# whh1747012859/Enhanced-UNet

Hardware: AMD Instinct MI355X
Metric: training images/sec at 1024×1024 1-ch→2-cls, 1/2/4/8 MI355X; Dice vs CPU ref (higher is better)
Workload: dtype bf16

## Files before the change

### enhanced-unet_amd/csrc/conv3x3.hip

```cpp
#include <algorithm>
#include <type_traits>

#include "common.h"

EUNET_DEBUG_UNIT(conv3x3)

namespace {

constexpr int BN = 64;
constexpr int NTHR = 256;
constexpr int B_UNITS = 4 * BN * 9;
constexpr int B_LDS_BYTES = B_UNITS * 16;

template <typename T> struct KCh { static constexpr int v = 4 * Vec16<T>::N; };

struct FwdArgs {
  const void* x; int N, H, W, xct, xco, cin;
  const float* isc; const float* ish; int iss;
  const void* wp; int cout_pad, nkc;
  const float* bias;
  void* y; int yct, yco, cout;
  float* stats; int tx, ty, ntiles;
  const void* by; int byct, byco;
  const float* bmean; const float* bistd; const float* bsc; const float* bsh;
// ... 610 lines not shown
      }
  #if CONV_STAMP
      st_ep[2 + 2 * pass] = conv_stamp();
  #endif
      if (pass + 1 < NPASS) __syncthreads();
    }
  }
  if (bnb) {
    float bs1[E], bs2[E];
#pragma unroll
    for (int e = 0; e < E; ++e) {
      float v1 = bp1[e >> 1][e & 1], v2 = bp2[e >> 1][e & 1];
      if constexpr (UPX == 8) {
        v1 += __int_as_float(__builtin_amdgcn_mov_dpp(__float_as_int(v1), 0x128, 0xF, 0xF, false));
        v2 += __int_as_float(__builtin_amdgcn_mov_dpp(__float_as_int(v2), 0x128, 0xF, 0xF, false));
      }
      bs1[e] = xor32_sum(xor16_sum(v1));
      bs2[e] = xor32_sum(xor16_sum(v2));
    }
    __syncthreads();
    float* r2 = (float*)smem;
    if (lane < UPX) {
#pragma unroll
      for (int e = 0; e < E; ++e) {
        r2[(wv * UPX + lane) * 2 * E + e] = bs1[e];
        r2[(wv * UPX + lane) * 2 * E + E + e] = bs2[e];
      }
    }
    __syncthreads();
    if (tid < 2 * BN) {
      const int which = tid / BN, cc = tid % BN, u = cc / E, e = cc % E;
      float t = 0.f;
#pragma unroll
      for (int w = 0; w < NW; ++w) t += r2[(w * UPX + u) * 2 * E + which * E + e];
      if (co0 + cc < a.cout) a.bpart[((long long)tile * 2 + which) * a.cout + co0 + cc] = t;
    }
  }
#if CONV_STAMP
  const unsigned long long st_e = conv_stamp();
  if (tid == 0 && blockIdx.x < STAMP_BLOCKS) {
    unsigned long long* o = g_conv_stamps + (size_t)blockIdx.x * STAMP_N;
    o[0] = st_t0;
    o[1] = st_e - st_t0;
    o[2] = st_stage;
    o[3] = st_mfma;
    o[4] = st_e - st_a;
    o[5] = st_ep[0] - st_a;
    o[6] = st_ep[1] - st_ep[0];
    o[7] = st_ep[2] - st_ep[1];
    o[8] = st_ep[3] - st_ep[2];
    o[9] = st_ep[4] - st_ep[3];
    o[10] = st_e - st_ep[4];
  }
#endif
}


template <typename T>
__device__ __forceinline__ void pack_elem(const float* w, int cout, int cin, int flip, T* wp, int cout_p, int cin_p,
                                          long long id) {
  constexpr int E = Vec16<T>::N, KC = KCh<T>::v;
  const int e = (int)(id % E);
  long long r = id / E;
  const int t = (int)(r % 9); r /= 9;
  const int o = (int)(r % cout_p); r /= cout_p;
  const int qq = (int)(r % 4);
  const int kc = (int)(r / 4);
  const int i = kc * KC + qq * E + e;
  float v = 0.f;
  if (!flip) {
    if (o < cout && i < cin) v = w[((long long)o * cin + i) * 9 + t];
  } else {
    if (o < cin && i < cout) v = w[((long long)i * cin + o) * 9 + (8 - t)];
  }
  Elem<T>::st(wp + id, v);
}

template <typename T>
__global__ void pack_kernel(const float* w, int cout, int cin, int flip, T* wp, int cout_p, int cin_p) {
  const long long id = (long long)blockIdx.x * blockDim.x + threadIdx.x;
  if (id < (long long)cin_p * cout_p * 9) pack_elem<T>(w, cout, cin, flip, wp, cout_p, cin_p, id);
}

struct PackBatch {
  eunet_pack_desc d[EUNET_PACK_MAX];
  int cout_p[EUNET_PACK_MAX], cin_p[EUNET_PACK_MAX];
  int bstart[EUNET_PACK_MAX + 1];
  int n;
};
template <typename T>
__global__ __launch_bounds__(256) void pack_many_kernel(PackBatch b) {
  constexpr int E = Vec16<T>::N, KC = KCh<T>::v;
  const int bid = blockIdx.x;
  int k = 0;
  for (int i = 1; i < b.n; ++i) k = bid >= b.bstart[i] ? i : k;
  const eunet_pack_desc& d = b.d[k];
  const int cout_p = b.cout_p[k];
  const long long u = (long long)(bid - b.bstart[k]) * 256 + threadIdx.x;
  if (u >= (long long)b.cin_p[k] * cout_p * 9 / E) return;
  long long r = u;
  const int t = (int)(r % 9); r /= 9;
  const int o = (int)(r % cout_p); r /= cout_p;
  const int qq = (int)(r % 4);
  const int kc = (int)(r / 4);
  const int i0 = kc * KC + qq * E;
  float v[E];
  bool ok[E];
#pragma unroll
  for (int e = 0; e < E; ++e) {
    const int i = i0 + e;
    ok[e] = d.flip ? (o < d.cin && i < d.cout) : (o < d.cout && i < d.cin);
    const long long src = !ok[e] ? 0 : d.flip ? ((long long)i * d.cin + o) * 9 + (8 - t) : ((long long)o * d.cin + i) * 9 + t;
    v[e] = d.w[src];
  }
#pragma unroll
  for (int e = 0; e < E; ++e) asm volatile("" : "+v"(v[e]));
#pragma unroll
  for (int e = 0; e < E; ++e) v[e] = ok[e] ? v[e] : 0.f;
  *(uint4*)((T*)d.wp + u * E) = Vec16<T>::pack(v);
}

struct WgArgs {
  const void* x; int N, H, W, xct, xco, cin;
  const float* isc; const float* ish; int iss;
  const void* dy; int dct, dco, cout;
  float* dw; float* db;
  int tx, ty, ntiles, per_split, nsplit;
};

__device__ __forceinline__ int wd_swz(int p) { return p & 6; }

__device__ __forceinline__ void wg_map(int b, int nsplit, int ncob, int ncib, int& split, int& cob, int& cib) {
  const int total = nsplit * ncob * ncib, full = total & ~7;
  const int L = b < full ? (b & 7) * (full >> 3) + (b >> 3) : b;
  cib = L % ncib;
  const int r = L / ncib;
  cob = r % ncob;
  split = r / ncob;
}

constexpr int KCW = 64;
constexpr int DTH = 8, DTW = 16;
constexpr int DHW = DTW + 2;
constexpr int DHPX = (DTH + 2) * DHW;
constexpr int DPL = 384;
constexpr int DWX = 4 * DPL * 16;
constexpr int DWD = DTH * DTW * 64 * 2;
constexpr int DSTAGE = DWX + DWD;
constexpr int DWX_ITERS = 4 * DPL / NTHR;
constexpr int DWD_ITERS = DTH * DTW * 8 / NTHR;
static_assert(4 * DPL == NTHR * DWX_ITERS && DTH * DTW * 8 == NTHR * DWD_ITERS, "whole wave-instructions");
static_assert(2 * DHPX <= DPL && DPL % 16 == 0, "a pair plane holds the halo, bank-row aligned");
static_assert(2 * DSTAGE <= 80 * 1024, "two stages per block, two blocks per CU");
static_assert(DPL > NTHR, "dma_x: one pair-plane boundary per wave-instruction range at most");

__device__ __forceinline__ void dma16_lds(u32x4 rsrc, uint32_t voff, uint32_t lds) {
  asm volatile("s_mov_b32 m0, %0\n\tbuffer_load_dwordx4 %1, %2, 0 offen lds"
               :: "s"(lds), "v"(voff), "s"(rsrc) : "memory", "m0");
}
__device__ __forceinline__ u32x4 rsrc_of(const void* base, uint32_t bytes) {
  const unsigned long long b = (unsigned long long)base;
  return (u32x4){(uint32_t)__builtin_amdgcn_readfirstlane((int)(uint32_t)b),
                 (uint32_t)__builtin_amdgcn_readfirstlane((int)(uint32_t)(b >> 32)),
                 (uint32_t)__builtin_amdgcn_readfirstlane((int)bytes), 0x00020000u};
}

__global__ __launch_bounds__(NTHR, 2) void conv3x3_wgrad_bf16_kernel(WgArgs a) {
  __shared__ __attribute__((aligned(16))) char wst[2 * DSTAGE];
  const int tid = threadIdx.x, lane = tid & 63, wv = tid >> 6;
  int split, cob, kc;
  wg_map(blockIdx.x, a.nsplit, cdiv(a.cout, 64), cdiv(a.cin, KCW), split, cob, kc);
  const int co0 = cob * 64;
  const int t_begin = split * a.per_split;
  const int t_end = min(a.ntiles, t_begin + a.per_split);
  EUNET_DASSERT(split < a.nsplit && co0 < a.cout && kc * KCW < a.cin && t_begin < a.ntiles);
  const int tpi = a.tx * a.ty;
  const int g = lane >> 4, i16 = lane & 15, q4 = i16 >> 2, p4 = i16 & 3;
  const int pcol = 4 * (g & 1) + q4;
  const int sw16 = (((p4 >> 1) ^ wd_swz(pcol)) * 8 + 4 * (p4 & 1)) * 2;

  f32x4 acc[9][4];
#pragma unroll
  for (int t = 0; t < 9; ++t)
#pragma unroll
    for (int c = 0; c < 4; ++c) acc[t][c] = (f32x4){0.f, 0.f, 0.f, 0.f};
  f32x2 dbv[4];
#pragma unroll
  for (int e = 0; e < 4; ++e) dbv[e] = (f32x2){0.f, 0.f};
  if (blockIdx.x & 1) __builtin_amdgcn_s_sleep(40);

  const uint32_t lds0 = (uint32_t)(size_t)(__attribute__((address_space(3))) char*)wst;
  const uint32_t wlds = lds0 + (uint32_t)__builtin_amdgcn_readfirstlane(wv) * 1024u;
  const int dp = tid >> 3, dcol = dp & (DTW - 1), drow = dp >> 4, du = (tid & 7) ^ wd_swz(dp);
  const bool dch_ok = co0 + du * 8 < a.cout;
  const uint32_t rstep = (uint32_t)(a.W * a.dct) * 2u;
  const uint32_t dlane = (uint32_t)((dcol * a.dct + a.dco + co0 + du * 8) * 2) + (uint32_t)drow * rstep;
  const uint32_t dslice = (uint32_t)(a.H * a.W * a.dct) * 2u, xslice = (uint32_t)(a.H * a.W * a.xct) * 2u;
  auto dma_d = [&](int st, int n, int y0, int x0) {
    const u32x4 dr = rsrc_of((const bf16_t*)a.dy + (long long)n * a.H * a.W * a.dct, dslice);
    const bool xok = dch_ok & (dcol < a.W - x0);
    const uint32_t rb = (uint32_t)((y0 * a.W + x0) * a.dct) * 2u;
    const uint32_t l = wlds + (uint32_t)(st * DSTAGE + DWX);
#pragma unroll
    for (int i = 0; i < DWD_ITERS; ++i) {
      const bool ok = xok & (y0 + 2 * i + drow < a.H);
      const uint32_t off = dlane + rb + 2u * i * rstep;
      EUNET_DASSERT(!ok || off + 16u <= dslice);
      dma16_lds(dr, ok ? off : FWD_OOB, l + 4096u * i);
    }
  };
  auto dma_x = [&](int st, int n, int y0, int x0) {
    const u32x4 xr = rsrc_of((const bf16_t*)a.x + (long long)n * a.H * a.W * a.xct, xslice);
    const int tb = ((y0 - 1) * a.W + (x0 - 1)) * a.xct + a.xco + kc * KCW;
    const uint32_t l = wlds + (uint32_t)(st * DSTAGE);
    int t = tid;
    asm volatile("" : "+v"(t));
#pragma unroll
    for (int i = 0; i < DWX_ITERS; ++i) {
      const int k = NTHR * i / DPL, tk = DPL * (k + 1) - NTHR * i;
      const bool bump = tk < NTHR && t >= tk;
      const int pr = k + bump, r = t + NTHR * i - DPL * pr;
      const int oc = 2 * pr + (r & 1), hp = r >> 1;
      const int hy = (int)((uint32_t)hp / DHW), hx = hp - hy * DHW;
      const bool ok = ((uint32_t)hp < (uint32_t)DHPX) & ((uint32_t)(y0 - 1 + hy) < (uint32_t)a.H) &
                      ((uint32_t)(x0 - 1 + hx) < (uint32_t)a.W) & (kc * KCW + oc * 8 < a.cin);
      const uint32_t off = (uint32_t)(tb + (hy * a.W + hx) * a.xct + oc * 8) * 2u;
      EUNET_DASSERT(!ok || off + 16u <= xslice);
      dma16_lds(xr, ok ? off : FWD_OOB, l + 4096u * i);
    }
  };
  const int xo = 2 * wv + (lane & 1);
  const bool xo_ok = kc * KCW + xo * 8 < a.cin;
  auto load_aff = [&](int n, f32x4* sc) {
    const float* ps = a.isc + (long long)n * a.iss + kc * KCW + xo * 8;
    const float* ph = a.ish + (long long)n * a.iss + kc * KCW + xo * 8;
    const f32x4 z = {0.f, 0.f, 0.f, 0.f};
    sc[0] = xo_ok ? *(const f32x4*)ps : z;
    sc[1] = xo_ok ? *(const f32x4*)(ps + 4) : z;
    sc[2] = xo_ok ? *(const f32x4*)ph : z;
    sc[3] = xo_ok ? *(const f32x4*)(ph + 4) : z;
  };
  auto bnrelu_x = [&](char* S, int y0, int x0, const f32x4* sc) {
    if (!xo_ok) return;
    const float scv[8] = {sc[0][0], sc[0][1], sc[0][2], sc[0][3], sc[1][0], sc[1][1], sc[1][2], sc[1][3]};
    const float shv[8] = {sc[2][0], sc[2][1], sc[2][2], sc[2][3], sc[3][0], sc[3][1], sc[3][2], sc[3][3]};
    char* const plane = S + (wv * DPL + lane) * 16;
    constexpr int G = 3, NI = (2 * DHPX + 63) / 64;
    static_assert(NI % G == 0, "bnrelu_x groups");
    static_assert((3 * DPL + 63 + 64 * (NI - 1) + 1) * 16 <= DSTAGE, "bnrelu_x: group reads stay inside the stage");
#pragma unroll 1
    for (int i0 = 0; i0 < NI; i0 += G) {
      u32x4 w[G];
      bool ok[G];
#pragma unroll
      for (int j = 0; j < G; ++j) {
        const int hp = (lane >> 1) + 32 * (i0 + j), hy = hp / DHW, hx = hp - hy * DHW;
        const int yy = y0 + hy - 1, xx = x0 + hx - 1;
        ok[j] = (hp < DHPX) & ((uint32_t)yy < (uint32_t)a.H) & ((uint32_t)xx < (uint32_t)a.W);
        w[j] = *(const u32x4*)(plane + 64 * (i0 + j) * 16);
      }
#pragma unroll
      for (int j = 0; j < G; ++j) {
        u32x4 o;
#pragma unroll
        for (int d = 0; d < 4; ++d) {
          const f32x2 x = {__uint_as_float(w[j][d] << 16), __uint_as_float(w[j][d] & 0xFFFF0000u)};
          const f32x2 r = __builtin_elementwise_fma(x, (f32x2){scv[2 * d], scv[2 * d + 1]}, (f32x2){shv[2 * d], shv[2 * d + 1]});
          const s16x2 b = __builtin_bit_cast(s16x2, pk_bf16(r[0], r[1]));
          o[d] = __builtin_bit_cast(uint32_t, __builtin_elementwise_max(b, (s16x2){0, 0}));
        }
        if (ok[j]) *(u32x4*)(plane + 64 * (i0 + j) * 16) = o;
      }
    }
  };
  int tn = t_begin / tpi, tyi = (t_begin - tn * tpi) / a.tx, txi = t_begin - tn * tpi - tyi * a.tx;
  const bool tf = a.isc != nullptr;
  {
    const int n = __builtin_amdgcn_readfirstlane(tn);
    dma_x(0, n, __builtin_amdgcn_readfirstlane(tyi) * DTH, __builtin_amdgcn_readfirstlane(txi) * DTW);
    dma_d(0, n, __builtin_amdgcn_readfirstlane(tyi) * DTH, __builtin_amdgcn_readfirstlane(txi) * DTW);
  }
  for (int tile = t_begin; tile < t_end; ++tile) {
    const int st = (tile - t_begin) & 1;
    char* const S = wst + st * DSTAGE;
    const int n = __builtin_amdgcn_readfirstlane(tn);
    const int y0 = __builtin_amdgcn_readfirstlane(tyi) * DTH, x0 = __builtin_amdgcn_readfirstlane(txi) * DTW;
    if (++txi == a.tx) {
      txi = 0;
      if (++tyi == a.ty) { tyi = 0; ++tn; }
    }
    f32x4 sc[4];
    if (tf) load_aff(n, sc);
    __builtin_amdgcn_s_waitcnt(0x0F70);
    __syncthreads();
    if (tile + 1 < t_end) {
      const int n1 = __builtin_amdgcn_readfirstlane(tn);
      const int y1 = __builtin_amdgcn_readfirstlane(tyi) * DTH, x1 = __builtin_amdgcn_readfirstlane(txi) * DTW;
      dma_x(st ^ 1, n1, y1, x1);
      dma_d(st ^ 1, n1, y1, x1);
    }
    if (tf) {
      bnrelu_x(S, y0, x0, sc);
      asm volatile("s_waitcnt lgkmcnt(0)" ::: "memory");
    }
    const char* const Xs = S;
    const char* const Ds = S + DWX;
    if (a.db != nullptr && kc == 0) {
      const bf16_t* d = (const bf16_t*)Ds;
#pragma unroll
      for (int i = 0; i < DTH * DTW / 32; ++i) {
        const int px = (tid >> 3) + 32 * i;
        const u32x4 w = *(const u32x4*)(d + px * 64 + ((tid & 7) ^ wd_swz(px)) * 8);
#pragma unroll
        for (int e = 0; e < 4; ++e) dbv[e] += (f32x2){__uint_as_float(w[e] << 16), __uint_as_float(w[e] & 0xFFFF0000u)};
      }
    }
    __builtin_amdgcn_s_setprio(1);
#pragma unroll 1
    for (int ks = 0; ks < DTH * DTW / 32; ++ks) {
      bf16x8 af[4];
      const int pxa = ks * 32 + 16 * (g >> 1) + pcol;
#pragma unroll
      for (int ct = 0; ct < 4; ++ct) {
        const int uo = (32 * ct) ^ sw16;
        const s16x4 lo = __builtin_amdgcn_ds_read_tr16_b64_v4i16(LDS_PTR(s16x4, Ds + pxa * 128 + uo));
        const s16x4 hi = __builtin_amdgcn_ds_read_tr16_b64_v4i16(LDS_PTR(s16x4, Ds + (pxa + 8) * 128 + uo));
        af[ct] = cat_bf16x4(lo, hi);
      }
      const int hrow = 2 * ks + (g >> 1);
#pragma unroll
      for (int t = 0; t < 9; ++t) {
        const int ky = t / 3, kx = t - ky * 3;
        const int hp = (hrow + ky) * DHW + pcol + kx;
        const char* base = Xs + (wv * DPL + 2 * hp + (p4 >> 1)) * 16 + (p4 & 1) * 8;
        const s16x4 lo = __builtin_amdgcn_ds_read_tr16_b64_v4i16(LDS_PTR(s16x4, base));
        const s16x4 hi = __builtin_amdgcn_ds_read_tr16_b64_v4i16(LDS_PTR(s16x4, base + 16 * 16));
        const bf16x8 bfr = cat_bf16x4(lo, hi);
#pragma unroll
        for (int ct = 0; ct < 4; ++ct)
          acc[t][ct] = __builtin_amdgcn_mfma_f32_16x16x32_bf16(af[ct], bfr, acc[t][ct], 0, 0, 0);
      }
    }
    __builtin_amdgcn_s_setprio(0);
  }
  float* out = a.dw + (long long)split * a.cout * 9 * a.cin;
  const int ci = kc * KCW + wv * 16 + i16;
#pragma unroll
  for (int t = 0; t < 9; ++t)
#pragma unroll
    for (int ct = 0; ct < 4; ++ct)
#pragma unroll
      for (int e = 0; e < 4; ++e) {
        const int co = co0 + ct * 16 + g * 4 + e;
        if (co < a.cout && ci < a.cin) {
          EUNET_DASSERT(split < a.nsplit);
          out[((long long)co * 9 + t) * a.cin + ci] = acc[t][ct][e];
        }
      }
  if (a.db != nullptr && kc == 0) {
    float* dbred = (float*)wst;
    __syncthreads();
#pragma unroll
    for (int e = 0; e < 8; ++e) dbred[(tid >> 3) * 64 + (tid & 7) * 8 + e] = dbv[e >> 1][e & 1];
    __syncthreads();
    if (tid < 64 && co0 + tid < a.cout) {
      float t = 0.f;
      for (int r = 0; r < 32; ++r) t += dbred[r * 64 + tid];
      a.db[(long long)split * a.cout + co0 + tid] = t;
    }
  }
}

constexpr int WF_TH = 4, WF_TW = 32;
constexpr int WF_HW = WF_TW + 2;
constexpr int WF_HP = (WF_TH + 2) * WF_HW;
constexpr int WF_CI = 32, WF_CO = 64;
constexpr int WF_XU = WF_HP * WF_CI / 4;
constexpr int WF_DU = WF_TH * WF_TW * WF_CO / 4;
constexpr int WF_XI = (WF_XU + NTHR - 1) / NTHR;
constexpr int WF_DI = WF_DU / NTHR;
constexpr int WF_XS = (WF_CI / 16) * WF_HP * 16;
constexpr int WF_LDS = (WF_XS + (WF_CO / 16) * WF_TH * WF_TW * 16 + 4 * 64) * 4;
static_assert(2 * WF_LDS <= 160 * 1024, "fp32 wgrad: two blocks per CU");

__global__ __launch_bounds__(NTHR, 2) void conv3x3_wgrad_f32_kernel(WgArgs a) {
  extern __shared__ __attribute__((aligned(16))) char smem[];
  float* Xs = (float*)smem;
  float* Ds = Xs + WF_XS;
  float* dbs = Ds + (WF_CO / 16) * WF_TH * WF_TW * 16;
  const int tid = threadIdx.x, lane = tid & 63, wv = tid >> 6;
  int split, cob, cib;
  wg_map(blockIdx.x, a.nsplit, cdiv(a.cout, WF_CO), cdiv(a.cin, WF_CI), split, cob, cib);
  const int co0 = cob * WF_CO, ci0 = cib * WF_CI;
  const int t_begin = split * a.per_split;
  const int t_end = min(a.ntiles, t_begin + a.per_split);
  const int tpi = a.tx * a.ty;
  const int kq = lane >> 4, li = lane & 15;
  const int ct0 = 2 * (wv >> 1), cit = wv & 1;
  const bool do_db = a.db != nullptr && cib == 0;

  f32x4 acc[2][9];
#pragma unroll
  for (int j = 0; j < 2; ++j)
#pragma unroll
    for (int t = 0; t < 9; ++t) acc[j][t] = (f32x4){0.f, 0.f, 0.f, 0.f};
  float dbacc = 0.f;

  uint4 rx[WF_XI], rd[WF_DI];
  unsigned rok = 0;
  auto gload = [&](int tile) {
    const int n = tile / tpi, trem = tile - n * tpi;
    const int y0 = (trem / a.tx) * WF_TH, x0 = (trem % a.tx) * WF_TW;
    rok = 0;
#pragma unroll
    for (int i = 0; i < WF_XI; ++i) {
      const int u = tid + i * NTHR;
      const int m = u & 3, hp = (u >> 2) % WF_HP, tl = (u >> 2) / WF_HP;
      const int hy = hp / WF_HW, hx = hp - hy * WF_HW;
      const int yy = y0 + hy - 1, xx = x0 + hx - 1, c = ci0 + tl * 16 + 4 * m;
      rx[i] = make_uint4(0, 0, 0, 0);
      if (u < WF_XU && yy >= 0 && yy < a.H && xx >= 0 && xx < a.W && c < a.cin) {
        rx[i] = *(const uint4*)((const float*)a.x + ((long long)(n * a.H + yy) * a.W + xx) * a.xct + a.xco + c);
        rok |= 1u << i;
      }
    }
#pragma unroll
    for (int i = 0; i < WF_DI; ++i) {
      const int u = tid + i * NTHR;
      const int m = u & 3, px = (u >> 2) % (WF_TH * WF_TW), tl = (u >> 2) / (WF_TH * WF_TW);
      const int yy = y0 + px / WF_TW, xx = x0 + px % WF_TW, co = co0 + tl * 16 + 4 * m;
      rd[i] = make_uint4(0, 0, 0, 0);
      if (yy < a.H && xx < a.W && co < a.cout)
        rd[i] = *(const uint4*)((const float*)a.dy + ((long long)(n * a.H + yy) * a.W + xx) * a.dct + a.dco + co);
    }
  };
  auto lwrite = [&](int tile) {
    const int n = tile / tpi;
#pragma unroll
    for (int i = 0; i < WF_XI; ++i) {
      const int u = tid + i * NTHR;
      if (u >= WF_XU) continue;
      uint4 v = rx[i];
      if (a.isc != nullptr && ((rok >> i) & 1u)) {
        const int m = u & 3, tl = (u >> 2) / WF_HP, c = ci0 + tl * 16 + 4 * m + n * a.iss;
        float f[4];
        Vec16<float>::unpack(v, f);
#pragma unroll
        for (int e = 0; e < 4; ++e) f[e] = fmaxf(fmaf(f[e], a.isc[c + e], a.ish[c + e]), 0.f);
        v = Vec16<float>::pack(f);
      }
      *(uint4*)(Xs + 4 * u) = v;
    }
#pragma unroll
    for (int i = 0; i < WF_DI; ++i) *(uint4*)(Ds + 4 * (tid + i * NTHR)) = rd[i];
  };

  if (t_begin < t_end) gload(t_begin);
  for (int tile = t_begin; tile < t_end; ++tile) {
    __syncthreads();
    lwrite(tile);
    __syncthreads();
    if (tile + 1 < t_end) gload(tile + 1);
    if (do_db) {
#pragma unroll 4
      for (int i = 0; i < WF_TH * WF_TW / 4; ++i) {
        const int px = (tid >> 6) + 4 * i, co = tid & 63;
        dbacc += Ds[((co >> 4) * WF_TH * WF_TW + px) * 16 + (co & 15)];
      }
    }
    const float* xb = Xs + cit * WF_HP * 16 + li;
    const float* d0 = Ds + (ct0 * WF_TH * WF_TW) * 16 + li;
    const float* d1 = d0 + WF_TH * WF_TW * 16;
#pragma unroll 2
    for (int ks = 0; ks < WF_TH * WF_TW / 4; ++ks) {
      const int px = 4 * ks + kq, r = px / WF_TW, c = px - r * WF_TW;
      const float a0 = d0[px * 16], a1 = d1[px * 16];
#pragma unroll
      for (int t = 0; t < 9; ++t) {
        const int ky = t / 3, kx = t - 3 * ky;
        const float bv = xb[((r + ky) * WF_HW + c + kx) * 16];
        acc[0][t] = __builtin_amdgcn_mfma_f32_16x16x4f32(a0, bv, acc[0][t], 0, 0, 0);
        acc[1][t] = __builtin_amdgcn_mfma_f32_16x16x4f32(a1, bv, acc[1][t], 0, 0, 0);
      }
    }
  }
  float* out = a.dw + (long long)split * a.cout * 9 * a.cin;
  const int ci = ci0 + cit * 16 + li;
#pragma unroll
  for (int j = 0; j < 2; ++j)
#pragma unroll
    for (int t = 0; t < 9; ++t)
#pragma unroll
      for (int i = 0; i < 4; ++i) {
        const int co = co0 + (ct0 + j) * 16 + 4 * kq + i;
        if (co < a.cout && ci < a.cin) out[((long long)co * 9 + t) * a.cin + ci] = acc[j][t][i];
// ... 291 lines not shown
```

### enhanced-unet_amd/eunet/engine.py

```python
from __future__ import annotations

from typing import Dict, Optional

import torch

from . import kprof, ops
from ._lib import EunetError

ENCODER_SCOPE = "conv3x3.encoder_train"

BLOCKS = ("enc1", "enc2", "enc3", "enc4", "dec4", "dec3", "dec2")
UPCONVS = ("up4", "up3", "up2")
BN_EPS = 1e-5
BN_MOMENTUM = 0.1
class Grad1x1:

    def __init__(self, w, k, gz):
        self.w, self.k, self.gz = w, k, gz


class GradPool:

    def __init__(self, gpool, gskip):
        self.gpool, self.gskip = gpool, gskip
# ... 127 lines not shown
        S = self.forward_trunk(x, training)
        P, B = self._P(), self._B()
        N, H, W, K, dev = S["N"], S["H"], S["W"], self.K, x.device
        z = S["z"]
        hws = _e(ops.head_workspace_bytes(N, H, W, K, self.dtype), torch.uint8, dev)
        hmean = _e(64, torch.float32, dev) if training else None
        hinv = _e(64, torch.float32, dev) if training else None
        out2h = _e((N, K, 2 * H, 2 * W), torch.float32, dev) if want == "out2h" else None
        logits = _e((N, K, H, W), torch.float32, dev) if want == "logits" else None
        ops.head_fwd(z, N, H, W, K, P["enhance.0.weight"], P["enhance.0.bias"], P["enhance.1.weight"],
                     P["enhance.1.bias"], P["enhance.3.weight"].reshape(K, 64).contiguous(), P["enhance.3.bias"],
                     training, BN_EPS, BN_MOMENTUM, B["enhance.1.running_mean"], B["enhance.1.running_var"],
                     hmean, hinv, out2h, logits, hws, dtype=self.dtype)
        if training:
            guard = ops.update_guard(dev)
            if guard is None:
                B["enhance.1.num_batches_tracked"].add_(1)
            else:
                B["enhance.1.num_batches_tracked"].add_(guard.eq(0).long().reshape(()))
        S.update(hmean=hmean, hinv=hinv, want=want)
        return (logits if want == "logits" else out2h), S

    def forward_trunk(self, x: torch.Tensor, training: bool):
        if not x.is_cuda:
            raise EunetError("EnhancedUNet (eunet) runs on the GPU only; no CPU fallback")
        N, Cin, H, W = x.shape
        if Cin != self.cin:
            raise ValueError(f"expected {self.cin} input channels, got {Cin}")
        if H % 8 or W % 8:
            raise ValueError("H and W must be multiples of 8 (the reference pads to /32)")
        P, B = self._P(), self._B()
        dt, dev, b, K = self.dtype, x.device, self.base, self.K
        ch = [b, 2 * b, 4 * b, 8 * b]
        lv = [(H >> i, W >> i) for i in range(4)]
        S = {}
        wps = self._pack_all(P, training)
        S["wp"] = wps
        if self.transpose:
            S["up"] = {u: ops.upconv2x2_pack(P[f"{self.prefix}{u}.weight"], dt) for u in UPCONVS}
        xin = _e((N, H, W, Cin), dt, dev)
        ops.nchw_to_nhwc(x.contiguous().float(), xin)
        cat4 = _e((N, *lv[2], ch[3] + ch[2]), dt, dev)
        cat3 = _e((N, *lv[1], ch[2] + ch[1]), dt, dev)
        cat2 = _e((N, *lv[0], ch[1] + ch[0]), dt, dev)
        p1 = _e((N, *lv[1], ch[0]), dt, dev)
        p2 = _e((N, *lv[2], ch[1]), dt, dev)
        p3 = _e((N, *lv[3], ch[2]), dt, dev)
        S.update(xin=xin, cat4=cat4, cat3=cat3, cat2=cat2, p1=p1, p2=p2, p3=p3)

        def consume_pool(nm, cat, coff, pooled):
            s = S[nm]
            ops.bnrelu_pool(ops.act(s["yb"]), s["bnb"]["scale"], s["bnb"]["shift"],
                            ops.act(cat, coff, s["yb"].shape[3]), ops.act(pooled))

        def consume_up(nm, cat, up):
            s = S[nm]
            if self.transpose:
                ops.bnrelu_upconv2x2(ops.act(s["yb"]), s["bnb"]["scale"], s["bnb"]["shift"], S["up"][up],
                                     P[f"{self.prefix}{up}.bias"], ops.act(cat, 0, s["yb"].shape[3]))
                return
            ops.bnrelu_upsample(ops.act(s["yb"]), s["bnb"]["scale"], s["bnb"]["shift"],
                                ops.act(cat, 0, s["yb"].shape[3]))

        S["enc1"] = self._block_fwd("enc1", ops.act(xin), training, P, B, small=True, wps=wps)
        consume_pool("enc1", cat2, ch[1], p1)
        S["enc2"] = self._block_fwd("enc2", ops.act(p1), training, P, B, small=False, wps=wps)
        consume_pool("enc2", cat3, ch[2], p2)
        S["enc3"] = self._block_fwd("enc3", ops.act(p2), training, P, B, small=False, wps=wps)
        consume_pool("enc3", cat4, ch[3], p3)
        S["enc4"] = self._block_fwd("enc4", ops.act(p3), training, P, B, small=False, wps=wps)
        consume_up("enc4", cat4, "up4")
        S["dec4"] = self._block_fwd("dec4", ops.act(cat4), training, P, B, small=False, wps=wps)
        consume_up("dec4", cat3, "up3")
        S["dec3"] = self._block_fwd("dec3", ops.act(cat3), training, P, B, small=False, wps=wps)
        consume_up("dec3", cat2, "up2")
        S["dec2"] = self._block_fwd("dec2", ops.act(cat2), training, P, B, small=False, wps=wps)
        s = S["dec2"]
        z = _e((N, H, W, K), torch.float32, dev)
        ops.bnrelu_conv1x1(ops.act(s["yb"]), s["bnb"]["scale"], s["bnb"]["shift"],
                           P[self.prefix + "dec1.weight"].reshape(K, b).contiguous(), P[self.prefix + "dec1.bias"], K, z)
        S.update(z=z, N=N, H=H, W=W)
        return S

    def _block_bwd(self, nm, G, S, P, sink, need_gx: bool, small: bool, gred=(None, 0)):
        with kprof.scope(ENCODER_SCOPE if nm.startswith("enc") else None):
            return self._block_bwd_impl(nm, G, S, P, sink, need_gx, small, gred)

    def _block_bwd_impl(self, nm, G: "torch.Tensor | Grad1x1 | GradPool", S, P, sink: GradSink, need_gx: bool,
                        small: bool, gred=(None, 0)):
        p = f"{self.prefix}{nm}"
        s = S[nm]
        ya, yb, bna, bnb, X = s["ya"], s["yb"], s["bna"], s["bnb"], s["X"]
        N, H, W, C = yb.shape
        dev, dt = yb.device, self.dtype

        def bn_back(prefix, g, y, bn, part=None, tiles=0):
            if isinstance(g, (Grad1x1, GradPool)):
                dbeta, dgamma = sink.slot(prefix + ".bias", (C,)), sink.slot(prefix + ".weight", (C,))
                ops.colsum(part, tiles, 2 * C, dbeta, split=C, out_hi=dgamma)
                gy = torch.empty_like(y)
                if isinstance(g, Grad1x1):
                    ops.bn_bwd_apply_1x1(ops.act(y), g.w, g.k, g.gz, bn["mean"], bn["invstd"], bn["scale"],
                                         bn["shift"], dbeta, dgamma, ops.act(gy))
                else:
                    ops.bn_bwd_apply_pool(g.gpool, g.gskip, ops.act(y), bn["mean"], bn["invstd"], bn["scale"],
                                          bn["shift"], dbeta, dgamma, ops.act(gy))
                return gy
            if part is None:
                tiles = ops.bn_bwd_tiles(ops.act(y))
                part = _e(tiles * 2 * C, torch.float32, dev)
                ops.bn_bwd_reduce(ops.act(g), ops.act(y), bn["mean"], bn["invstd"], bn["scale"],
                                  bn["shift"], part)
            dbeta, dgamma = sink.slot(prefix + ".bias", (C,)), sink.slot(prefix + ".weight", (C,))
            ops.colsum(part, tiles, 2 * C, dbeta, split=C, out_hi=dgamma)
            gy = torch.empty_like(y)
            ops.bn_bwd_apply(ops.act(g), ops.act(y), bn["mean"], bn["invstd"], bn["scale"],
                             bn["shift"], dbeta, dgamma, ops.act(gy))
            return gy

        main = torch.cuda.current_stream(dev)
        side = side_stream(dev) if self.overlap_wgrad else None

        def wgrad(conv, xa: ops.Act, gy, scale=None, shift=None, small_conv=False, on_main=False):
            dw = sink.slot(conv + ".weight", (C, xa.c, 3, 3))
            db = sink.slot(conv + ".bias", (C,))
            if side is None or on_main:
                return wgrad_on_stream(xa, gy, dw, db, scale, shift, small_conv)
            self._wait(side, main)
            with torch.cuda.stream(side):
                wgrad_on_stream(xa, gy, dw, db, scale, shift, small_conv)
            for t in (gy, xa._keep, dw, db):
                t.record_stream(side)

        def wgrad_on_stream(xa: ops.Act, gy, dw, db, scale=None, shift=None, small_conv=False):
            cin = xa.c
            gya = ops.act(gy)
            if small_conv:
                ns = ops.conv_small_wgrad_splits(gya)
            else:
                ns = ops.conv3x3_wgrad_splits(gya, cin, dt)
            dwp = _e(ns * C * 9 * cin, torch.float32, dev)
            dbp = _e(ns * C, torch.float32, dev)
            if small_conv:
                ops.conv_small_wgrad(xa, gya, dwp, dbp, ns)
            else:
                ops.conv3x3_wgrad(xa, gya, dwp, dbp, ns, scale=scale, shift=shift)
            ops.wgrad_reduce(dwp, dbp, ns, C, cin, 9, dw, db)

        def packed(conv):
            wpt = S["wp"].get(conv + ".weight^T") if S.get("wp") else None
            return wpt if wpt is not None else ops.conv3x3_pack(P[conv + ".weight"], dt, flip=True)

        gyb = bn_back(p + ".4", G, yb, bnb, part=gred[0], tiles=gred[1])
        wpt = packed(p + ".3")
        gaa = torch.empty_like(ya)
        ctiles = ops.conv3x3_tiles(ops.act(gaa))
        cpart = _e(ctiles * 2 * C, torch.float32, dev)
        ops.conv3x3_dgrad_bnbwd(ops.act(gyb), wpt, ops.act(gaa), ops.act(ya), bna["mean"], bna["invstd"],
                                bna["scale"], bna["shift"], cpart)
        gya = bn_back(p + ".1", gaa, ya, bna, part=cpart, tiles=ctiles)
        if s.get("za") is not None:
            wgrad(p + ".3", ops.act(s["za"]), gyb)
        else:
            wgrad(p + ".3", ops.act(ya), gyb, bna["scale"], bna["shift"])
        del gyb
        wgrad(p + ".0", X, gya, small_conv=small, on_main=not need_gx)
        del gaa
        names = [f"{p}.{i}.{w}" for i in (0, 1, 3, 4) for w in ("weight", "bias")]
        if side is None:
            sink.ready(names)
        else:
            self._wait(side, main)
            with torch.cuda.stream(side):
                sink.ready(names)
        if not need_gx:
            return None
        wpt = packed(p + ".0")
        gx = _e((N, H, W, X.c), dt, dev)
        ops.conv3x3_dgrad(ops.act(gya), wpt, ops.act(gx))
        return gx

    def backward(self, S, g_out: torch.Tensor, sink: Optional[GradSink] = None):
        P = self._P()
        N, H, W, K, b = S["N"], S["H"], S["W"], self.K, self.base
        dev, dt = g_out.device, self.dtype
        ch = [b, 2 * b, 4 * b, 8 * b]
        sink = sink or GradSink(dev)
        g_out = g_out.contiguous().float()
        gz = _e((N, H, W, K), torch.float32, dev)
        hws = _e(ops.head_workspace_bytes(N, H, W, K, dt), torch.uint8, dev)
        gw1 = sink.slot("enhance.0.weight", (64, K, 3, 3))
        gb1 = sink.slot("enhance.0.bias", (64,))
        gg = sink.slot("enhance.1.weight", (64,))
        gbt = sink.slot("enhance.1.bias", (64,))
        gw2 = sink.slot("enhance.3.weight", (K, 64, 1, 1))
        gb2 = sink.slot("enhance.3.bias", (K,))
        glog = g_out if S["want"] == "logits" else None
        gout2h = g_out if S["want"] == "out2h" else None
        ops.head_bwd(S["z"], N, H, W, K, P["enhance.0.weight"], P["enhance.0.bias"], P["enhance.1.weight"],
                     P["enhance.1.bias"], P["enhance.3.weight"].reshape(K, 64).contiguous(), S["hmean"], S["hinv"],
                     glog, gout2h, gz, gw1, gb1, gg, gbt, gw2, gb2, hws, dtype=dt)
        sink.ready(["enhance.0.weight", "enhance.0.bias", "enhance.1.weight", "enhance.1.bias",
                    "enhance.3.weight", "enhance.3.bias"])
        self.backward_trunk(S, gz, sink)
        return sink.finish()

    def backward_trunk(self, S, gz: torch.Tensor, sink: GradSink):
        P = self._P()
        N, H, W, K, b = S["N"], S["H"], S["W"], self.K, self.base
        dev, dt = gz.device, self.dtype
        ch = [b, 2 * b, 4 * b, 8 * b]
        pre = self.prefix

        def bnr_args(nm):
            s = S[nm]
            return (ops.act(s["yb"]), s["bnb"]["mean"], s["bnb"]["invstd"], s["bnb"]["scale"], s["bnb"]["shift"])

        def upconv_bwd(ghi: ops.Act, glo: torch.Tensor, nm, up):
            s = S[nm]
            C = glo.shape[3]
            ops.upconv2x2_dgrad(ghi, S["up"][up], ops.act(glo))
            names = [f"{pre}{up}.weight", f"{pre}{up}.bias"]
            dw, db = sink.slot(names[0], (C, C, 2, 2)), sink.slot(names[1], (C,))

            def wgrad():
                ya = ops.act(s["yb"])
                ns = ops.upconv2x2_wgrad_splits(ya, dt)
                dwp = _e(ns * 4 * C * C, torch.float32, dev)
                dbp = _e(ns * 4 * C, torch.float32, dev)
                ops.upconv2x2_wgrad(ya, s["bnb"]["scale"], s["bnb"]["shift"], ghi, dwp, dbp, ns)
                ops.wgrad_reduce(dwp, None, ns, C, C, 4, dw, None)
                ops.colsum(dbp, ns * 4, C, db)
                sink.ready(names)

            if not self.overlap_wgrad:
                wgrad()
                return None, 0
            main, side = torch.cuda.current_stream(dev), side_stream(dev)
            self._wait(side, main)
            with torch.cuda.stream(side):
                wgrad()
            for t in (ghi._keep, s["yb"], dw, db):
                t.record_stream(side)
            return None, 0

        def up_bwd(ghi: ops.Act, glo: torch.Tensor, nm, up):
            if self.transpose:
                return upconv_bwd(ghi, glo, nm, up)
            rows = ops.upsample_bwd_bnr_rows(ops.act(glo))
            if not rows:
                ops.upsample_bwd(ghi, ops.act(glo))
                return None, 0
            part = _e(rows * 2 * glo.shape[3], torch.float32, dev)
            ops.upsample_bwd_bnr(ghi, ops.act(glo), *bnr_args(nm), part)
            return part, rows

        def pool_bwd(act_saved: ops.Act, gpool: ops.Act, gskip: ops.Act, shape, nm):
            rows = ops.pool_bwd_add_bnr_rows(act_saved)
            if not rows:
                gout = _e(shape, dt, dev)
                ops.pool_bwd_add(act_saved, gpool, gskip, ops.act(gout))
                return gout, (None, 0)
            part = _e(rows * 2 * shape[3], torch.float32, dev)
            if self.pool_recompute:
                ops.pool_bwd_add_bnr(act_saved, gpool, gskip, None, *bnr_args(nm), part)
                return GradPool(gpool, gskip), (part, rows)
            gout = _e(shape, dt, dev)
            ops.pool_bwd_add_bnr(act_saved, gpool, gskip, ops.act(gout), *bnr_args(nm), part)
            return gout, (part, rows)

        s2 = S["dec2"]
        yb_act = ops.act(s2["yb"])
        tiles = ops.conv1x1_bwd_tiles(yb_act)
        part = _e(tiles * (K * b + K), torch.float32, dev)
        w1 = P[pre + "dec1.weight"].reshape(K, b).contiguous()
        bnb2 = s2["bnb"]
        bpart = _e(tiles * 2 * b, torch.float32, dev)
        if self.dec1_recompute:
            gd2 = Grad1x1(w1, K, gz)
            ops.conv1x1_bwd_bnr(yb_act, bnb2["scale"], bnb2["shift"], w1, K, gz, None, part,
                                bnb2["mean"], bnb2["invstd"], bpart)
        else:
            gd2 = torch.empty_like(s2["yb"])
            ops.conv1x1_bwd_bnr(yb_act, bnb2["scale"], bnb2["shift"], w1, K, gz, ops.act(gd2), part,
                                bnb2["mean"], bnb2["invstd"], bpart)
        red2 = (bpart, tiles)
        ops.colsum(part, tiles, K * b + K, sink.slot(pre + "dec1.weight", (K, b, 1, 1)), split=K * b,
                   out_hi=sink.slot(pre + "dec1.bias", (K,)))
        sink.ready([pre + "dec1.weight", pre + "dec1.bias"])
        g_cat2 = self._block_bwd("dec2", gd2, S, P, sink, need_gx=True, small=False, gred=red2)
        del gd2
        g_d3 = _e((N, H >> 1, W >> 1, ch[1]), dt, dev)
        red = up_bwd(ops.act(g_cat2, 0, ch[1]), g_d3, "dec3", "up2")
        g_cat3 = self._block_bwd("dec3", g_d3, S, P, sink, need_gx=True, small=False, gred=red)
        del g_d3
        g_d4 = _e((N, H >> 2, W >> 2, ch[2]), dt, dev)
        red = up_bwd(ops.act(g_cat3, 0, ch[2]), g_d4, "dec4", "up3")
        g_cat4 = self._block_bwd("dec4", g_d4, S, P, sink, need_gx=True, small=False, gred=red)
        del g_d4
        g_e4 = _e((N, H >> 3, W >> 3, ch[3]), dt, dev)
        red = up_bwd(ops.act(g_cat4, 0, ch[3]), g_e4, "enc4", "up4")
        g_p3 = self._block_bwd("enc4", g_e4, S, P, sink, need_gx=True, small=False, gred=red)
        del g_e4
        g_e3, red = pool_bwd(ops.act(S["cat4"], ch[3], ch[2]), ops.act(g_p3), ops.act(g_cat4, ch[3], ch[2]),
                             (N, H >> 2, W >> 2, ch[2]), "enc3")
        del g_p3, g_cat4
        g_p2 = self._block_bwd("enc3", g_e3, S, P, sink, need_gx=True, small=False, gred=red)
        del g_e3
        g_e2, red = pool_bwd(ops.act(S["cat3"], ch[2], ch[1]), ops.act(g_p2), ops.act(g_cat3, ch[2], ch[1]),
                             (N, H >> 1, W >> 1, ch[1]), "enc2")
        del g_p2, g_cat3
        g_p1 = self._block_bwd("enc2", g_e2, S, P, sink, need_gx=True, small=False, gred=red)
        del g_e2
        g_e1, red = pool_bwd(ops.act(S["cat2"], ch[1], ch[0]), ops.act(g_p1), ops.act(g_cat2, ch[1], ch[0]),
                             (N, H, W, ch[0]), "enc1")
        del g_p1, g_cat2
        self._block_bwd("enc1", g_e1, S, P, sink, need_gx=False, small=True, gred=red)
# ... 24 lines not shown
```

Measured before the change: 192.8.

## Reuse halo rows across vertically consecutive wgrad tiles and reorder tile walk

The conv3x3 wgrad kernel now walks tiles column-major (down y first), so consecutive tiles share two halo rows. Those rows are no longer re-DMA'd or re-normalised, and the top-row input fragments are carried in registers between k-steps and across tiles. Each wave now copies its own pair plane, a separate BN-ReLU path skips bounds checks for interior tiles, and the engine issues one wgrad earlier when no input gradient is needed. The aim is to cut global loads, LDS reads and BN-ReLU work, at the cost of more live registers and more complex correctness conditions.

```diff
diff --git a/enhanced-unet_amd/csrc/conv3x3.hip b/enhanced-unet_amd/csrc/conv3x3.hip
--- a/enhanced-unet_amd/csrc/conv3x3.hip
+++ b/enhanced-unet_amd/csrc/conv3x3.hip
@@ -786,7 +786,8 @@
 static_assert(4 * DPL == NTHR * DWX_ITERS && DTH * DTW * 8 == NTHR * DWD_ITERS, "whole wave-instructions");
 static_assert(2 * DHPX <= DPL && DPL % 16 == 0, "a pair plane holds the halo, bank-row aligned");
 static_assert(2 * DSTAGE <= 80 * 1024, "two stages per block, two blocks per CU");
-static_assert(DPL > NTHR, "dma_x: one pair-plane boundary per wave-instruction range at most");
+static_assert(DPL == 64 * DWX_ITERS, "dma_x: a wave copies its own pair plane in whole wave-instructions");
+static_assert(2 * 2 * DHW >= 64 && 2 * 2 * DHW < 128, "dma_x: halo rows 0, 1 end inside wave-instruction 1");
 
 __device__ __forceinline__ void dma16_lds(u32x4 rsrc, uint32_t voff, uint32_t lds) {
   asm volatile("s_mov_b32 m0, %0\n\tbuffer_load_dwordx4 %1, %2, 0 offen lds"
@@ -843,24 +844,25 @@
       dma16_lds(dr, ok ? off : FWD_OOB, l + 4096u * i);
     }
   };
-  auto dma_x = [&](int st, int n, int y0, int x0) {
+  auto dma_x = [&](int st, int n, int y0, int x0, bool start) {
     const u32x4 xr = rsrc_of((const bf16_t*)a.x + (long long)n * a.H * a.W * a.xct, xslice);
     const int tb = ((y0 - 1) * a.W + (x0 - 1)) * a.xct + a.xco + kc * KCW;
-    const uint32_t l = wlds + (uint32_t)(st * DSTAGE);
-    int t = tid;
+    const uint32_t l = lds0 + (uint32_t)(st * DSTAGE) + (uint32_t)__builtin_amdgcn_readfirstlane(wv) * (DPL * 16u);
+    const int hp_min = start ? 0 : 2 * DHW;
+    int t = lane;
     asm volatile("" : "+v"(t));
+    const int oc = 2 * wv + (t & 1);
 #pragma unroll
     for (int i = 0; i < DWX_ITERS; ++i) {
-      const int k = NTHR * i / DPL, tk = DPL * (k + 1) - NTHR * i;
-      const bool bump = tk < NTHR && t >= tk;
-      const int pr = k + bump, r = t + NTHR * i - DPL * pr;
-      const int oc = 2 * pr + (r & 1), hp = r >> 1;
+      if (i == 0 && !start) continue;
+      const int hp = (t >> 1) + 32 * i;
       const int hy = (int)((uint32_t)hp / DHW), hx = hp - hy * DHW;
-      const bool ok = ((uint32_t)hp < (uint32_t)DHPX) & ((uint32_t)(y0 - 1 + hy) < (uint32_t)a.H) &
+      const bool ok = (hp >= hp_min) & ((uint32_t)hp < (uint32_t)DHPX) & ((uint32_t)(y0 - 1 + hy) < (uint32_t)a.H) &
                       ((uint32_t)(x0 - 1 + hx) < (uint32_t)a.W) & (kc * KCW + oc * 8 < a.cin);
       const uint32_t off = (uint32_t)(tb + (hy * a.W + hx) * a.xct + oc * 8) * 2u;
       EUNET_DASSERT(!ok || off + 16u <= xslice);
-      dma16_lds(xr, ok ? off : FWD_OOB, l + 4096u * i);
+      EUNET_DASSERT(l + 1024u * i + 1024u <= lds0 + (uint32_t)(st * DSTAGE + DWX));
+      dma16_lds(xr, ok ? off : FWD_OOB, l + 1024u * i);
     }
   };
   const int xo = 2 * wv + (lane & 1);
@@ -874,24 +876,29 @@
     sc[2] = xo_ok ? *(const f32x4*)ph : z;
     sc[3] = xo_ok ? *(const f32x4*)(ph + 4) : z;
   };
-  auto bnrelu_x = [&](char* S, int y0, int x0, const f32x4* sc) {
-    if (!xo_ok) return;
+  auto bnrelu_rows = [&](char* S, int y0, int x0, const f32x4* sc, bool start, auto inside) {
     const float scv[8] = {sc[0][0], sc[0][1], sc[0][2], sc[0][3], sc[1][0], sc[1][1], sc[1][2], sc[1][3]};
     const float shv[8] = {sc[2][0], sc[2][1], sc[2][2], sc[2][3], sc[3][0], sc[3][1], sc[3][2], sc[3][3]};
     char* const plane = S + (wv * DPL + lane) * 16;
     constexpr int G = 3, NI = (2 * DHPX + 63) / 64;
     static_assert(NI % G == 0, "bnrelu_x groups");
     static_assert((3 * DPL + 63 + 64 * (NI - 1) + 1) * 16 <= DSTAGE, "bnrelu_x: group reads stay inside the stage");
+    const int hp_min = start ? 0 : 2 * DHW;
 #pragma unroll 1
     for (int i0 = 0; i0 < NI; i0 += G) {
       u32x4 w[G];
       bool ok[G];
 #pragma unroll
       for (int j = 0; j < G; ++j) {
-        const int hp = (lane >> 1) + 32 * (i0 + j), hy = hp / DHW, hx = hp - hy * DHW;
-        const int yy = y0 + hy - 1, xx = x0 + hx - 1;
-        ok[j] = (hp < DHPX) & ((uint32_t)yy < (uint32_t)a.H) & ((uint32_t)xx < (uint32_t)a.W);
-        w[j] = *(const u32x4*)(plane + 64 * (i0 + j) * 16);
+        const int hp = (lane >> 1) + 32 * (i0 + j);
+        ok[j] = (hp >= hp_min) & (hp < DHPX);
+        if (!decltype(inside)::value) {
+          const int hy = hp / DHW, hx = hp - hy * DHW;
+          const int yy = y0 + hy - 1, xx = x0 + hx - 1;
+          ok[j] &= ((uint32_t)yy < (uint32_t)a.H) & ((uint32_t)xx < (uint32_t)a.W);
+        }
+        w[j] = (u32x4){0u, 0u, 0u, 0u};
+        if (start || i0 + j > 0) w[j] = *(const u32x4*)(plane + 64 * (i0 + j) * 16);
       }
 #pragma unroll
       for (int j = 0; j < G; ++j) {
@@ -907,21 +914,28 @@
       }
     }
   };
-  int tn = t_begin / tpi, tyi = (t_begin - tn * tpi) / a.tx, txi = t_begin - tn * tpi - tyi * a.tx;
+  auto bnrelu_x = [&](char* S, int y0, int x0, const f32x4* sc, bool start) {
+    if (!xo_ok) return;
+    if (y0 >= 1 && y0 + DTH < a.H && x0 >= 1 && x0 + DTW < a.W) bnrelu_rows(S, y0, x0, sc, start, std::true_type{});
+    else bnrelu_rows(S, y0, x0, sc, start, std::false_type{});
+  };
+  int tn = t_begin / tpi, txi = (t_begin - tn * tpi) / a.ty, tyi = t_begin - tn * tpi - txi * a.ty;
   const bool tf = a.isc != nullptr;
   {
     const int n = __builtin_amdgcn_readfirstlane(tn);
-    dma_x(0, n, __builtin_amdgcn_readfirstlane(tyi) * DTH, __builtin_amdgcn_readfirstlane(txi) * DTW);
+    dma_x(0, n, __builtin_amdgcn_readfirstlane(tyi) * DTH, __builtin_amdgcn_readfirstlane(txi) * DTW, true);
     dma_d(0, n, __builtin_amdgcn_readfirstlane(tyi) * DTH, __builtin_amdgcn_readfirstlane(txi) * DTW);
   }
+  bf16x8 cf[3], c1[3];
   for (int tile = t_begin; tile < t_end; ++tile) {
     const int st = (tile - t_begin) & 1;
     char* const S = wst + st * DSTAGE;
     const int n = __builtin_amdgcn_readfirstlane(tn);
     const int y0 = __builtin_amdgcn_readfirstlane(tyi) * DTH, x0 = __builtin_amdgcn_readfirstlane(txi) * DTW;
-    if (++txi == a.tx) {
-      txi = 0;
-      if (++tyi == a.ty) { tyi = 0; ++tn; }
+    const bool start = tile == t_begin || y0 == 0;
+    if (++tyi == a.ty) {
+      tyi = 0;
+      if (++txi == a.tx) { txi = 0; ++tn; }
     }
     f32x4 sc[4];
     if (tf) load_aff(n, sc);
@@ -930,15 +944,28 @@
     if (tile + 1 < t_end) {
       const int n1 = __builtin_amdgcn_readfirstlane(tn);
       const int y1 = __builtin_amdgcn_readfirstlane(tyi) * DTH, x1 = __builtin_amdgcn_readfirstlane(txi) * DTW;
-      dma_x(st ^ 1, n1, y1, x1);
+      dma_x(st ^ 1, n1, y1, x1, y1 == 0);
       dma_d(st ^ 1, n1, y1, x1);
     }
     if (tf) {
-      bnrelu_x(S, y0, x0, sc);
+      bnrelu_x(S, y0, x0, sc, start);
       asm volatile("s_waitcnt lgkmcnt(0)" ::: "memory");
     }
     const char* const Xs = S;
     const char* const Ds = S + DWX;
+    const char* const xlane = Xs + (wv * DPL + 2 * pcol + (p4 >> 1)) * 16 + (p4 & 1) * 8;
+    auto xfrag = [&](const char* base) {
+      const s16x4 lo = __builtin_amdgcn_ds_read_tr16_b64_v4i16(LDS_PTR(s16x4, base));
+      const s16x4 hi = __builtin_amdgcn_ds_read_tr16_b64_v4i16(LDS_PTR(s16x4, base + 16 * 16));
+      return cat_bf16x4(lo, hi);
+    };
+    if (start) {
+#pragma unroll
+      for (int kx = 0; kx < 3; ++kx) {
+        cf[kx] = xfrag(xlane + (((g >> 1) * DHW + kx) * 2) * 16);
+        c1[kx] = xfrag(xlane + ((DHW + kx) * 2) * 16);
+      }
+    }
     if (a.db != nullptr && kc == 0) {
       const bf16_t* d = (const bf16_t*)Ds;
 #pragma unroll
@@ -949,9 +976,7 @@
         for (int e = 0; e < 4; ++e) dbv[e] += (f32x2){__uint_as_float(w[e] << 16), __uint_as_float(w[e] & 0xFFFF0000u)};
       }
     }
-    __builtin_amdgcn_s_setprio(1);
-#pragma unroll 1
-    for (int ks = 0; ks < DTH * DTW / 32; ++ks) {
+    auto kstep = [&](int ks, auto first) {
       bf16x8 af[4];
       const int pxa = ks * 32 + 16 * (g >> 1) + pcol;
 #pragma unroll
@@ -961,20 +986,29 @@
         const s16x4 hi = __builtin_amdgcn_ds_read_tr16_b64_v4i16(LDS_PTR(s16x4, Ds + (pxa + 8) * 128 + uo));
         af[ct] = cat_bf16x4(lo, hi);
       }
-      const int hrow = 2 * ks + (g >> 1);
+      const char* const xrow = xlane + ((2 * ks + (g >> 1)) * DHW * 2) * 16;
 #pragma unroll
       for (int t = 0; t < 9; ++t) {
         const int ky = t / 3, kx = t - ky * 3;
-        const int hp = (hrow + ky) * DHW + pcol + kx;
-        const char* base = Xs + (wv * DPL + 2 * hp + (p4 >> 1)) * 16 + (p4 & 1) * 8;
-        const s16x4 lo = __builtin_amdgcn_ds_read_tr16_b64_v4i16(LDS_PTR(s16x4, base));
-        const s16x4 hi = __builtin_amdgcn_ds_read_tr16_b64_v4i16(LDS_PTR(s16x4, base + 16 * 16));
-        const bf16x8 bfr = cat_bf16x4(lo, hi);
+        bf16x8 bfr;
+        if (ky == 0) {
+          bfr = cf[kx];
+        } else {
+          bfr = xfrag(xrow + ((ky * DHW + kx) * 2) * 16);
+          if (decltype(first)::value && ky == 1) bfr = lane < 32 ? c1[kx] : bfr;
+          if (ky == 2) cf[kx] = bfr;
+        }
 #pragma unroll
         for (int ct = 0; ct < 4; ++ct)
           acc[t][ct] = __builtin_amdgcn_mfma_f32_16x16x32_bf16(af[ct], bfr, acc[t][ct], 0, 0, 0);
       }
-    }
+    };
+    __builtin_amdgcn_s_setprio(1);
+    kstep(0, std::true_type{});
+#pragma unroll 1
+    for (int ks = 1; ks < DTH * DTW / 32; ++ks) kstep(ks, std::false_type{});
+#pragma unroll
+    for (int kx = 0; kx < 3; ++kx) c1[kx] = xfrag(xlane + (((DTH + 1) * DHW + kx) * 2) * 16);
     __builtin_amdgcn_s_setprio(0);
   }
   float* out = a.dw + (long long)split * a.cout * 9 * a.cin;
diff --git a/enhanced-unet_amd/eunet/engine.py b/enhanced-unet_amd/eunet/engine.py
--- a/enhanced-unet_amd/eunet/engine.py
+++ b/enhanced-unet_amd/eunet/engine.py
@@ -303,6 +303,15 @@
             return wpt if wpt is not None else ops.conv3x3_pack(P[conv + ".weight"], dt, flip=True)
 
         gyb = bn_back(p + ".4", G, yb, bnb, part=gred[0], tiles=gred[1])
+
+        def wgrad3():
+            if s.get("za") is not None:
+                wgrad(p + ".3", ops.act(s["za"]), gyb)
+            else:
+                wgrad(p + ".3", ops.act(ya), gyb, bna["scale"], bna["shift"])
+
+        if not need_gx:
+            wgrad3()
         wpt = packed(p + ".3")
         gaa = torch.empty_like(ya)
         ctiles = ops.conv3x3_tiles(ops.act(gaa))
@@ -310,10 +319,8 @@
         ops.conv3x3_dgrad_bnbwd(ops.act(gyb), wpt, ops.act(gaa), ops.act(ya), bna["mean"], bna["invstd"],
                                 bna["scale"], bna["shift"], cpart)
         gya = bn_back(p + ".1", gaa, ya, bna, part=cpart, tiles=ctiles)
-        if s.get("za") is not None:
-            wgrad(p + ".3", ops.act(s["za"]), gyb)
-        else:
-            wgrad(p + ".3", ops.act(ya), gyb, bna["scale"], bna["shift"])
+        if need_gx:
+            wgrad3()
         del gyb
         wgrad(p + ".0", X, gya, small_conv=small, on_main=not need_gx)
         del gaa
```

Result: no change. 192.7, median of 2 (-0.1%).
